# crmorton/Turbo-Whisper-Workspace

Hardware: AMD Instinct MI355X
Metric: real-time factor (audio-sec/wall-sec) Whisper-v3-turbo, 30s chunks, 1/2/4/8 GPU (higher is better)
Workload: dtype bf16; 1 GPU; whisper-large-v3-turbo bf16, batch=24 x 30s windows per GPU, greedy, 128 new tokens/window (EOS suppressed, one seek pass), timestamps on, language detected; collectives=none, global_batch=24, seq_len=3000, parallelism=chunk-dp1

## Files before the change

### turbo-whisper-workspace_amd/csrc/gemm.hip

```cpp
#include <algorithm>
#include <type_traits>

#include "tw_common.h"
#include "../../include/tw_whisper.h"

struct EpiArgs {
  void* out;
  int ldo;
  const float* bias;
  const float* aux;
  int aux_rows;
  int kv_S, kv_B, kv_D, kv_H;
  uint8_t* sout;
  int s_rows;
  int group_m;
};

__device__ inline void tw_tile_grouped(int wgid, int ntm, int ntn, int gm, int& tm, int& tn) {
  if (gm <= 1) {
    tm = wgid / ntn;
    tn = wgid - tm * ntn;
    return;
  }
  const int per = gm * ntn, g = wgid / per, first = g * gm;
// ... 222 lines not shown
        }
        continue;
      }
#pragma unroll
      for (int rr = 0; rr < 16; ++rr) {
        const int lr = rr * 4 + (lane >> 4);
        const int m = mrow0 + lr;
        float4 v = *(const float4*)(wimg + lr * GB_EPI_LD + rc);
        v.x += bias4.x; v.y += bias4.y; v.z += bias4.z; v.w += bias4.w;
        if (full) {
          if (m < M) epi_store4_pre<EPI>(ea, m, ncol0 + rc, v, ad[rr & 7]);
        } else if (m < M && ncol0 + rc < N) {
          epi_store4<EPI>(ea, m, ncol0 + rc, N, v);
        }
        if (rr < 8) ad[rr] = epi_addend<EPI>(ea, min(m + 32, M - 1), ncol0 + rc, full);
      }
    } else if constexpr (EPI == TW_EPI_BF16 || EPI == TW_EPI_GELU_BF16 || EPI == TW_EPI_CROSSKV) {
      const int rc8 = (lane & 7) * 8;
#pragma unroll 4
      for (int rr = 0; rr < 8; ++rr) {
        const int lr = rr * 8 + (lane >> 3);
        const int m = mrow0 + lr;
        float4 v0 = *(const float4*)(wimg + lr * GB_EPI_LD + rc8);
        float4 v1 = *(const float4*)(wimg + lr * GB_EPI_LD + rc8 + 4);
        v0.x += b8[0]; v0.y += b8[1]; v0.z += b8[2]; v0.w += b8[3];
        v1.x += b8[4]; v1.y += b8[5]; v1.z += b8[6]; v1.w += b8[7];
        if (m < M && ncol0 + rc8 < N) epi_store8<EPI>(ea, m, ncol0 + rc8, N, v0, v1);
      }
    } else {
#pragma unroll 4
      for (int rr = 0; rr < 16; ++rr) {
        const int lr = rr * 4 + (lane >> 4);
        const int m = mrow0 + lr;
        float4 v = *(const float4*)(wimg + lr * GB_EPI_LD + rc);
        v.x += bias4.x; v.y += bias4.y; v.z += bias4.z; v.w += bias4.w;
        if (m < M && ncol0 + rc < N) epi_store4<EPI>(ea, m, ncol0 + rc, N, v);
      }
    }
  }
}

template <int EPI>
__device__ inline void gemm_epi_128x64(const f32x4 (&acc)[8][4], float* wimg, int lane, int mw0, int ncol0, int M,
                                       int N, const EpiArgs& ea, bool interior = false) {
  const int fr = lane & 15, fq = lane >> 4;
  auto stage = [&](int half, float* w) {
    const int ib = 4 * half;
#pragma unroll
    for (int ii = 0; ii < 4; ++ii)
#pragma unroll
      for (int j = 0; j < 4; ++j)
#pragma unroll
        for (int r = 0; r < 4; ++r) w[(ii * 16 + fq * 4 + r) * GB_EPI_LD + j * 16 + fr] = acc[ib + ii][j][r];
  };
  gemm_epi_128x64_st<EPI>(stage, wimg, lane, mw0, ncol0, M, N, ea, interior);
}
template <int EPI, class Acc, class RowMap, class TCol>
__device__ inline void gemm_epi_tr(Acc acc, bf16_t* img, const float* bias_s, int lane, RowMap rowmap, TCol tcol, int n0,
                                   int M, int N, const EpiArgs& ea) {
  const int fr = lane & 15, fq = lane >> 4;
  float4 b4[4];
#pragma unroll
  for (int j = 0; j < 4; ++j)
    b4[j] = ea.bias ? *(const float4*)(bias_s + tcol(16 * j + 4 * fq)) : make_float4(0.f, 0.f, 0.f, 0.f);
  if constexpr (EPI == TW_EPI_BF16 || EPI == TW_EPI_GELU_BF16 || EPI == TW_EPI_CROSSKV) {
#pragma unroll
    for (int i = 0; i < 8; ++i) {
      const int row = 16 * i + fr;
#pragma unroll
      for (int j = 0; j < 4; ++j) {
        const f32x4 a = acc(i, j);
        float4 v = make_float4(a[0] + b4[j].x, a[1] + b4[j].y, a[2] + b4[j].z, a[3] + b4[j].w);
        if constexpr (EPI == TW_EPI_GELU_BF16) v = gelu_erf4(v);
        uint2 w;
        w.x = pack_bf16x2(v.x, v.y);
        w.y = pack_bf16x2(v.z, v.w);
        *(uint2*)(img + row * 64 + (((4 * j + fq) ^ (row & 15)) << 2)) = w;
      }
    }
    gb_epi_sync();
#pragma unroll 4
    for (int rr = 0; rr < 16; ++rr) {
      const int row = rr * 8 + (lane >> 3), p = lane & 7, g = row & 15;
      uint4 d = *(const uint4*)(img + row * 64 + ((p ^ (g >> 1)) << 3));
      if (g & 1) d = make_uint4(d.z, d.w, d.x, d.y);
      const int m = rowmap(row), n = n0 + tcol(8 * p);
      if (m >= M || n >= N) continue;
      if (n + 7 < N) {
        size_t idx;
        if constexpr (EPI == TW_EPI_CROSSKV) {
          const int D = ea.kv_D, S = ea.kv_S;
          const int l = n / (2 * D), rem = n - l * 2 * D;
          const int kv = rem / D, hd = rem - kv * D;
          const int b = m / S, s2 = m - b * S;
          idx = ((((size_t)(l * 2 + kv) * ea.kv_B + b) * ea.kv_H + (hd >> 6)) * S + s2) * 64 + (hd & 63);
        } else {
          idx = (size_t)m * ea.ldo + n;
        }
        tw_st_enc<gb_nt_bit(EPI)>((bf16_t*)ea.out + idx, d);
      } else {
        const uint32_t u[4] = {d.x, d.y, d.z, d.w};
        EpiArgs e2 = ea;
        e2.bias = nullptr;
        for (int e = 0; e < 8 && n + e < N; ++e) {
          const bf16_t h = (bf16_t)((u[e >> 1] >> (16 * (e & 1))) & 0xffffu);
          if constexpr (EPI == TW_EPI_CROSSKV) {
            epi_store<EPI>(e2, m, n + e, bf16_to_f32(h));
          } else {
            ((bf16_t*)ea.out)[(size_t)m * ea.ldo + n + e] = h;
          }
        }
      }
    }
  } else {
    constexpr bool PRE = EPI == TW_EPI_RESID_F32 || EPI == TW_EPI_GELU_POS_F32;
    float4 ad[2][4];
    auto load_ad = [&](int i, float4 (&dst)[4]) {
      const int m = min(rowmap(16 * i + fr), M - 1);
#pragma unroll
      for (int j = 0; j < 4; ++j) {
        const int n = n0 + tcol(16 * j + 4 * fq);
        dst[j] = epi_addend<EPI>(ea, m, n, n + 3 < N);
      }
    };
    if constexpr (PRE) load_ad(0, ad[0]);
#pragma unroll
    for (int i = 0; i < 8; ++i) {
      if constexpr (PRE) {
        if (i + 1 < 8) load_ad(i + 1, ad[(i + 1) & 1]);
      }
      const int m = rowmap(16 * i + fr);
#pragma unroll
      for (int j = 0; j < 4; ++j) {
        const f32x4 a = acc(i, j);
        const float4 v = make_float4(a[0] + b4[j].x, a[1] + b4[j].y, a[2] + b4[j].z, a[3] + b4[j].w);
        const int n = n0 + tcol(16 * j + 4 * fq);
        if (m >= M || n >= N) continue;
        if (n + 3 < N) {
          if constexpr (PRE) epi_store4_pre<EPI>(ea, m, n, v, ad[i & 1][j]);
          else epi_store4<EPI>(ea, m, n, N, v);
        } else {
          epi_store4<EPI>(ea, m, n, N, v);
        }
      }
    }
  }
}

__device__ inline void gemm_bias_load(const EpiArgs& ea, int n0, int N, float4& b) {
  const int c = n0 + 4 * (threadIdx.x & 63);
  if (ea.bias)
    b = make_float4(ea.bias[min(c, N - 1)], ea.bias[min(c + 1, N - 1)], ea.bias[min(c + 2, N - 1)],
                    ea.bias[min(c + 3, N - 1)]);
}

template <int EPI, bool TR>
__global__ __launch_bounds__(512, 1) void k_gemm_big(const bf16_t* __restrict__ A, const bf16_t* __restrict__ W,
                                                     int M, int N, int K, int lda, int ldw, EpiArgs ea) {
  __shared__ __attribute__((aligned(16))) bf16_t smem[8 * 64 * GB_EPI_LD * 2];
  const int tid = threadIdx.x, lane = tid & 63, wid = tid >> 6;
  const int ntm = (M + GB_BM - 1) / GB_BM, ntn = (N + GB_BN - 1) / GB_BN;
  const int nwg = ntm * ntn;
  const int orig = blockIdx.x;
  const int q8 = nwg / 8, r8 = nwg % 8, xcd = orig % 8;
  const int wgid = (xcd < r8 ? xcd * (q8 + 1) : r8 * (q8 + 1) + (xcd - r8) * q8) + orig / 8;
  int tm, tn;
  tw_tile_grouped(wgid, ntm, ntn, ea.group_m, tm, tn);
  const int m0 = tm * GB_BM, n0 = tn * GB_BN;

  const bf16_t* ga[4];
  const bf16_t* gw[4];
#pragma unroll
  for (int i = 0; i < 4; ++i) {
    const int row = 8 * (4 * wid + i) + (lane >> 3);
    const int ch = (lane & 7) ^ gb_swz(row);
    ga[i] = A + (size_t)min(m0 + row, M - 1) * lda + ch * 8;
    gw[i] = W + (size_t)min(n0 + row, N - 1) * ldw + ch * 8;
  }
  auto stage = [&](int buf, int k0) {
    bf16_t* As = smem + buf * 2 * GB_BM * GB_BK;
    bf16_t* Ws = As + GB_BM * GB_BK;
#pragma unroll
    for (int i = 0; i < 4; ++i) {
      const int rb = 8 * (4 * wid + i) * GB_BK;
      __builtin_amdgcn_global_load_lds((const void*)(ga[i] + k0), (lds_void_t*)(As + rb), 16, 0, 0);
      __builtin_amdgcn_global_load_lds((const void*)(gw[i] + k0), (lds_void_t*)(Ws + rb), 16, 0, 0);
    }
  };

  const int wr = wid >> 2, wc = wid & 3;
  const int fr = lane & 15, fq = lane >> 4;
  f32x4 acc[8][4];
#pragma unroll
  for (int i = 0; i < 8; ++i)
#pragma unroll
    for (int j = 0; j < 4; ++j) acc[i][j] = (f32x4){0.f, 0.f, 0.f, 0.f};

  const int nk = K / GB_BK;
  float* bias_s = (float*)(smem + 4 * GB_BM * GB_BK);
  float4 bl = make_float4(0.f, 0.f, 0.f, 0.f);
  stage(0, 0);
  if (TR && wid == 0) gemm_bias_load(ea, n0, N, bl);
  if (TR && wid == 0) {
    asm volatile("s_waitcnt vmcnt(0)" ::: "memory");
    *(float4*)(bias_s + 4 * lane) = bl;
  }
  __syncthreads();
  for (int kt = 0; kt < nk; ++kt) {
    const int cur = kt & 1;
    if (kt + 1 < nk) stage(cur ^ 1, (kt + 1) * GB_BK);
    const bf16_t* As = smem + cur * 2 * GB_BM * GB_BK;
    const bf16_t* Ws = As + GB_BM * GB_BK;
#pragma unroll
    for (int kk = 0; kk < 2; ++kk) {
      const int kc = 4 * kk + fq;
      bf16x8 bfr[4];
#pragma unroll
      for (int j = 0; j < 4; ++j) {
        const int col = wc * 64 + j * 16 + fr;
        bfr[j] = *(const bf16x8*)(Ws + col * GB_BK + ((kc ^ gb_swz(col)) << 3));
      }
#pragma unroll
      for (int i = 0; i < 8; ++i) {
        const int row = wr * 128 + i * 16 + fr;
        const bf16x8 af = *(const bf16x8*)(As + row * GB_BK + ((kc ^ gb_swz(row)) << 3));
#pragma unroll
        for (int j = 0; j < 4; ++j) {
          if constexpr (TR) acc[i][j] = __builtin_amdgcn_mfma_f32_16x16x32_bf16(bfr[j], af, acc[i][j], 0, 0, 0);
          else acc[i][j] = __builtin_amdgcn_mfma_f32_16x16x32_bf16(af, bfr[j], acc[i][j], 0, 0, 0);
        }
      }
    }
    __syncthreads();
  }

  if constexpr (TR) {
    gemm_epi_tr<EPI>([&](int i, int j) { return acc[i][j]; }, smem + wid * (128 * 64), bias_s, lane,
                     [&](int lr) { return m0 + wr * 128 + lr; }, [&](int lc) { return wc * 64 + lc; }, n0, M, N, ea);
  } else {
    gemm_epi_128x64<EPI>(acc, (float*)smem + wid * (64 * GB_EPI_LD), lane, m0 + wr * 128, n0 + wc * 64, M, N, ea,
                         m0 + GB_BM <= M && n0 + GB_BN <= N);
  }
}

__device__ inline __amdgpu_buffer_rsrc_t tw_uniform_rsrc(const void* p, int bytes) {
  const unsigned long long a = (unsigned long long)p;
  const unsigned lo = __builtin_amdgcn_readfirstlane((unsigned)a), hi = __builtin_amdgcn_readfirstlane((unsigned)(a >> 32));
  return __builtin_amdgcn_make_buffer_rsrc((void*)(((unsigned long long)hi << 32) | lo), 0,
                                           __builtin_amdgcn_readfirstlane(bytes), 0x00020000);
}

#ifdef TW_GEMM_PROBE
#define TW_PROBE_SLOTS 16
__device__ unsigned long long tw_probe_ts[32768 * TW_PROBE_SLOTS];
#define TW_PROBE(slot)                                                                                     \
  do {                                                                                                     \
    if (threadIdx.x == 0) tw_probe_ts[blockIdx.x * TW_PROBE_SLOTS + (slot)] = __builtin_amdgcn_s_memrealtime(); \
  } while (0)
#define TW_PROBE_CLK(slot)                                                                                 \
  do {                                                                                                     \
    if (threadIdx.x == 0) tw_probe_ts[blockIdx.x * TW_PROBE_SLOTS + (slot)] = __builtin_amdgcn_s_memtime();  \
  } while (0)
__device__ inline void tw_probe_ids() {
  if (threadIdx.x == 0) {
    unsigned hw, xcc;
    asm volatile("s_getreg_b32 %0, hwreg(HW_REG_HW_ID)" : "=s"(hw));
    asm volatile("s_getreg_b32 %0, hwreg(HW_REG_XCC_ID)" : "=s"(xcc));
    tw_probe_ts[blockIdx.x * TW_PROBE_SLOTS + 6] = hw;
    tw_probe_ts[blockIdx.x * TW_PROBE_SLOTS + 7] = xcc;
  }
}
extern "C" int tw_gemm_probe_read(unsigned long long* host, int nwg) {
  return (int)hipMemcpyFromSymbol(host, HIP_SYMBOL(tw_probe_ts), (size_t)nwg * TW_PROBE_SLOTS * 8, 0,
                                  hipMemcpyDeviceToHost);
}
#define TW_PROBE_W(slot)                              \
  do {                                                \
    asm volatile("s_waitcnt vmcnt(0) lgkmcnt(0)" ::: "memory"); \
    TW_PROBE(slot);                                   \
  } while (0)
#define TW_PROBE_END()                                \
  do {                                                \
    asm volatile("s_waitcnt vmcnt(0)" ::: "memory"); \
    __syncthreads();                                  \
    TW_PROBE(3);                                      \
  } while (0)
#else
#define TW_PROBE(slot) do {} while (0)
#define TW_PROBE_CLK(slot) do {} while (0)
#define TW_PROBE_END() do {} while (0)
#define TW_PROBE_W(slot) do {} while (0)
__device__ inline void tw_probe_ids() {}
#endif

template <int N>
__device__ inline void p8_vmcnt() {
  if constexpr (N == 0) asm volatile("s_waitcnt vmcnt(0)" ::: "memory");
  else if constexpr (N == 2) asm volatile("s_waitcnt vmcnt(2)" ::: "memory");
  else if constexpr (N == 4) asm volatile("s_waitcnt vmcnt(4)" ::: "memory");
  else if constexpr (N == 5) asm volatile("s_waitcnt vmcnt(5)" ::: "memory");
  else static_assert(N == 0, "unsupported vmcnt");
}

template <int EPI, bool TR>
__global__ __launch_bounds__(512, 1) void k_gemm_8p(const bf16_t* __restrict__ A, const bf16_t* __restrict__ W,
                                                    int M, int N, int K, int lda, int ldw, EpiArgs ea) {
  __shared__ __attribute__((aligned(16))) bf16_t smem[8 * 64 * GB_EPI_LD * 2];
  constexpr int HT = 128 * GB_BK;
  TW_PROBE(0);
  TW_PROBE_CLK(4);
  tw_probe_ids();
  const int tid = threadIdx.x, lane = tid & 63, wid = tid >> 6;
  const int ntm = (M + GB_BM - 1) / GB_BM, ntn = (N + GB_BN - 1) / GB_BN;
  const int nwg = ntm * ntn;
  const int orig = blockIdx.x;
  const int q8 = nwg / 8, r8 = nwg % 8, xcd = orig % 8;
  const int wgid = (xcd < r8 ? xcd * (q8 + 1) : r8 * (q8 + 1) + (xcd - r8) * q8) + orig / 8;
  int tm, tn;
  tw_tile_grouped(wgid, ntm, ntn, ea.group_m, tm, tn);
  const int m0 = tm * GB_BM, n0 = tn * GB_BN;
  const int wr = wid >> 2, wc = wid & 3;
  const int fr = lane & 15, fq = lane >> 4;

  __amdgpu_buffer_rsrc_t rs[4];
#pragma unroll
  for (int h = 0; h < 4; ++h) {
    const int r0 = (h < 2 ? m0 : n0) + 128 * (h & 1), lim = h < 2 ? M : N, ld = h < 2 ? lda : ldw;
    const int rows = max(0, min(128, lim - r0));
    rs[h] = tw_uniform_rsrc((h < 2 ? A : W) + (size_t)r0 * ld, rows ? ((rows - 1) * ld + K) * 2 : 0);
  }
  unsigned voff[2][2];
#pragma unroll
  for (int i = 0; i < 2; ++i) {
    const int row = 8 * (2 * wid + i) + (lane >> 3);
    const int ch = (lane & 7) ^ gb_swz(row);
    voff[0][i] = (unsigned)(row * lda + ch * 8) * 2u;
    voff[1][i] = (unsigned)(row * ldw + ch * 8) * 2u;
  }
  auto stage = [&](int buf, int h, int k0) {
    bf16_t* dst = smem + (buf * 4 + h) * HT;
#pragma unroll
    for (int i = 0; i < 2; ++i)
      __builtin_amdgcn_raw_ptr_buffer_load_lds(rs[h], (lds_void_t*)(dst + 8 * (2 * wid + i) * GB_BK), 16,
                                               voff[h >> 1][i], (unsigned)k0 * 2u, 0, 0);
  };

  bf16x8 af[4][2], bfr[2][2];
  auto readA = [&](int buf, int mh) {
    const bf16_t* As = smem + (buf * 4 + mh) * HT;
#pragma unroll
    for (int i = 0; i < 4; ++i)
#pragma unroll
      for (int kk = 0; kk < 2; ++kk) {
        const int row = 64 * wr + 16 * i + fr, kc = 4 * kk + fq;
        af[i][kk] = *(const bf16x8*)(As + row * GB_BK + ((kc ^ gb_swz(row)) << 3));
      }
  };
  auto readB = [&](int buf, int nh) {
    const bf16_t* Bs = smem + (buf * 4 + 2 + nh) * HT;
#pragma unroll
    for (int j = 0; j < 2; ++j)
#pragma unroll
      for (int kk = 0; kk < 2; ++kk) {
        const int row = 32 * wc + 16 * j + fr, kc = 4 * kk + fq;
        bfr[j][kk] = *(const bf16x8*)(Bs + row * GB_BK + ((kc ^ gb_swz(row)) << 3));
      }
  };
  f32x4 acc[2][2][4][2];
#pragma unroll
  for (int a = 0; a < 2; ++a)
#pragma unroll
    for (int b = 0; b < 2; ++b)
#pragma unroll
      for (int i = 0; i < 4; ++i)
#pragma unroll
        for (int j = 0; j < 2; ++j) acc[a][b][i][j] = (f32x4){0.f, 0.f, 0.f, 0.f};
  auto mfma_q = [&](auto MH, auto NH) {
    constexpr int mh = decltype(MH)::value, nh = decltype(NH)::value;
    __builtin_amdgcn_s_barrier();
    asm volatile("s_waitcnt lgkmcnt(0)" ::: "memory");
    __builtin_amdgcn_s_setprio(1);
#pragma unroll
    for (int kk = 0; kk < 2; ++kk)
#pragma unroll
      for (int i = 0; i < 4; ++i)
#pragma unroll
        for (int j = 0; j < 2; ++j)
          acc[mh][nh][i][j] = TR ? __builtin_amdgcn_mfma_f32_16x16x32_bf16(bfr[j][kk], af[i][kk], acc[mh][nh][i][j], 0, 0, 0)
                                 : __builtin_amdgcn_mfma_f32_16x16x32_bf16(af[i][kk], bfr[j][kk], acc[mh][nh][i][j], 0, 0, 0);
    __builtin_amdgcn_s_setprio(0);
    __builtin_amdgcn_s_barrier();
  };
  using I0 = std::integral_constant<int, 0>;
  using I1 = std::integral_constant<int, 1>;

  const int nk = K / GB_BK;
  float* bias_s = (float*)(smem + 8 * HT);
  float4 bl = make_float4(0.f, 0.f, 0.f, 0.f);
#pragma unroll
  for (int h = 0; h < 4; ++h) stage(0, h, 0);
  if (TR && wid == 0) gemm_bias_load(ea, n0, N, bl);
  asm volatile("s_waitcnt vmcnt(0)" ::: "memory");
  if (TR && wid == 0) *(float4*)(bias_s + 4 * lane) = bl;
  if (TR) asm volatile("s_waitcnt lgkmcnt(0)" ::: "memory");
  __builtin_amdgcn_s_barrier();
  TW_PROBE(1);
  if (wr == 1) __builtin_amdgcn_s_barrier();
  auto ktile = [&](int t, auto NXT) {
    constexpr bool nxt = decltype(NXT)::value;
    const int buf = t & 1, nb = buf ^ 1, kn = (t + 1) * GB_BK;
    readB(buf, 0);
    __builtin_amdgcn_sched_barrier(0);
    readA(buf, 0);
    if constexpr (nxt) {
      stage(nb, 0, kn);
      p8_vmcnt<4>();
    } else {
      p8_vmcnt<2>();
    }
    mfma_q(I0{}, I0{});
    readB(buf, 1);
    if constexpr (nxt) {
      stage(nb, 2, kn);
      p8_vmcnt<4>();
    } else {
      p8_vmcnt<0>();
    }
    mfma_q(I0{}, I1{});
    readA(buf, 1);
    if constexpr (nxt) stage(nb, 3, kn);
    mfma_q(I1{}, I1{});
    readB(buf, 0);
    if constexpr (nxt) {
      stage(nb, 1, kn);
      p8_vmcnt<4>();
    }
    mfma_q(I1{}, I0{});
  };
  using BT = std::integral_constant<bool, true>;
  using BF = std::integral_constant<bool, false>;
  for (int t = 0; t + 1 < nk; ++t) ktile(t, BT{});
  ktile(nk - 1, BF{});
  if (wr == 0) __builtin_amdgcn_s_barrier();
  __syncthreads();
  TW_PROBE(2);
  TW_PROBE_CLK(5);
  if constexpr (TR) {
    TW_PROBE_W(8);
    gemm_epi_tr<EPI>([&](int i, int j) { return acc[i >> 2][j >> 1][i & 3][j & 1]; }, smem + wid * (128 * 64), bias_s,
                     lane, [&](int lr) { return m0 + 128 * (lr >> 6) + 64 * wr + (lr & 63); },
                     [&](int lc) { return 128 * (lc >> 5) + 32 * wc + (lc & 31); }, n0, M, N, ea);
    TW_PROBE_END();
    return;
  }

  const int rc = (lane & 7) * 8;
  const int ncol = n0 + (rc < 32 ? 32 * wc + rc : 128 + 32 * wc + rc - 32);
  float4 b0 = make_float4(0.f, 0.f, 0.f, 0.f), b1 = b0;
  if (ea.bias) {
    b0.x = ea.bias[min(ncol, N - 1)];
    b0.y = ea.bias[min(ncol + 1, N - 1)];
    b0.z = ea.bias[min(ncol + 2, N - 1)];
    b0.w = ea.bias[min(ncol + 3, N - 1)];
    b1.x = ea.bias[min(ncol + 4, N - 1)];
    b1.y = ea.bias[min(ncol + 5, N - 1)];
    b1.z = ea.bias[min(ncol + 6, N - 1)];
    b1.w = ea.bias[min(ncol + 7, N - 1)];
  }
  float* wimg = (float*)smem + wid * (64 * GB_EPI_LD);
  TW_PROBE_W(8);
  constexpr bool PRE = EPI == TW_EPI_RESID_F32 || EPI == TW_EPI_GELU_POS_F32;
  const bool full = ncol + 7 < N;
#pragma unroll
  for (int mh = 0; mh < 2; ++mh) {
    const int mrow0 = m0 + 128 * mh + 64 * wr;
    float4 ad[4][2];
    if constexpr (PRE) {
#pragma unroll
      for (int q = 0; q < 4; ++q) {
        const int mq = min(mrow0 + q * 8 + (lane >> 3), M - 1);
        ad[q][0] = epi_addend<EPI>(ea, mq, ncol, full);
        ad[q][1] = epi_addend<EPI>(ea, mq, ncol + 4, full);
      }
    }
    if (mh) gb_epi_sync();
#pragma unroll
    for (int i = 0; i < 4; ++i)
#pragma unroll
      for (int nh = 0; nh < 2; ++nh)
#pragma unroll
        for (int j = 0; j < 2; ++j)
#pragma unroll
          for (int r = 0; r < 4; ++r)
            wimg[(i * 16 + fq * 4 + r) * GB_EPI_LD + nh * 32 + j * 16 + fr] = acc[mh][nh][i][j][r];
    gb_epi_sync();
    TW_PROBE_W(9 + 2 * mh);
#pragma unroll
    for (int rr = 0; rr < 8; ++rr) {
      const int lr = rr * 8 + (lane >> 3);
      const int m = mrow0 + lr;
      float4 v0 = *(const float4*)(wimg + lr * GB_EPI_LD + rc);
      float4 v1 = *(const float4*)(wimg + lr * GB_EPI_LD + rc + 4);
      v0.x += b0.x; v0.y += b0.y; v0.z += b0.z; v0.w += b0.w;
      v1.x += b1.x; v1.y += b1.y; v1.z += b1.z; v1.w += b1.w;
      if constexpr (PRE) {
        if (full) {
          if (m < M) {
            epi_store4_pre<EPI>(ea, m, ncol, v0, ad[rr & 3][0]);
            epi_store4_pre<EPI>(ea, m, ncol + 4, v1, ad[rr & 3][1]);
          }
        } else if (m < M && ncol < N) {
          epi_store8<EPI>(ea, m, ncol, N, v0, v1);
        }
        if (rr < 4) {
          const int mq = min(m + 32, M - 1);
          ad[rr][0] = epi_addend<EPI>(ea, mq, ncol, full);
          ad[rr][1] = epi_addend<EPI>(ea, mq, ncol + 4, full);
        }
      } else {
        if (m < M && ncol < N) epi_store8<EPI>(ea, m, ncol, N, v0, v1);
      }
    }
    TW_PROBE_W(10 + 2 * mh);
  }
  TW_PROBE_END();
}

__device__ inline void gb_read_rows4(const float* img, float4 (&v)[4][2]) {
  const unsigned a = (unsigned)(uintptr_t)(const __attribute__((address_space(3))) float*)img;
  asm volatile(
      "ds_read_b128 %0, %8\n\tds_read_b128 %1, %8 offset:16\n\t"
      "ds_read_b128 %2, %8 offset:%9\n\tds_read_b128 %3, %8 offset:%10\n\t"
      "ds_read_b128 %4, %8 offset:%11\n\tds_read_b128 %5, %8 offset:%12\n\t"
      "ds_read_b128 %6, %8 offset:%13\n\tds_read_b128 %7, %8 offset:%14\n\t"
      "s_waitcnt lgkmcnt(0)"
      : "=v"(v[0][0]), "=v"(v[0][1]), "=v"(v[1][0]), "=v"(v[1][1]), "=v"(v[2][0]), "=v"(v[2][1]), "=v"(v[3][0]),
        "=v"(v[3][1])
      : "v"(a), "i"(8 * GB_EPI_LD * 4), "i"(8 * GB_EPI_LD * 4 + 16), "i"(16 * GB_EPI_LD * 4),
        "i"(16 * GB_EPI_LD * 4 + 16), "i"(24 * GB_EPI_LD * 4), "i"(24 * GB_EPI_LD * 4 + 16)
      : "memory");
}

template <int EPI>
__global__ __launch_bounds__(512, 1) void k_gemm_8pp(const bf16_t* __restrict__ A, const bf16_t* __restrict__ W,
                                                     int M, int N, int K, int lda, int ldw, EpiArgs ea) {
  __shared__ __attribute__((aligned(16))) bf16_t smem[8 * 64 * GB_EPI_LD * 2];
  constexpr int HT = 128 * GB_BK;
  const int tid = threadIdx.x, lane = tid & 63, wid = tid >> 6;
  const int ntm = (M + GB_BM - 1) / GB_BM, ntn = (N + GB_BN - 1) / GB_BN;
  const int nwg = ntm * ntn;
  const int xcd = blockIdx.x % 8, slot = blockIdx.x / 8, S = gridDim.x / 8;
  const int q8 = nwg / 8, r8 = nwg % 8;
  const int cnt = q8 + (xcd < r8 ? 1 : 0);
  const int base = xcd < r8 ? xcd * (q8 + 1) : r8 * (q8 + 1) + (xcd - r8) * q8;
  if (slot >= cnt) return;
  const int wr = wid >> 2, wc = wid & 3;
  const int fr = lane & 15, fq = lane >> 4;
  float* const bias_sl = (float*)(smem + 4 * HT) + 8 * 32 * GB_EPI_LD;

  __amdgpu_buffer_rsrc_t rs[4];
  auto set_tile = [&](int tile, int& m0, int& n0) {
    int tm, tn;
    tw_tile_grouped(tile, ntm, ntn, ea.group_m, tm, tn);
    m0 = tm * GB_BM;
    n0 = tn * GB_BN;
#pragma unroll
    for (int h = 0; h < 4; ++h) {
      const int r0 = (h < 2 ? m0 : n0) + 128 * (h & 1), lim = h < 2 ? M : N, ld = h < 2 ? lda : ldw;
      const int rows = max(0, min(128, lim - r0));
      rs[h] = tw_uniform_rsrc((h < 2 ? A : W) + (size_t)r0 * ld, rows ? ((rows - 1) * ld + K) * 2 : 0);
    }
  };
  unsigned voff[2][2];
#pragma unroll
  for (int i = 0; i < 2; ++i) {
    const int row = 8 * (2 * wid + i) + (lane >> 3);
    const int ch = (lane & 7) ^ gb_swz(row);
    voff[0][i] = (unsigned)(row * lda + ch * 8) * 2u;
    voff[1][i] = (unsigned)(row * ldw + ch * 8) * 2u;
  }
  auto stage = [&](int buf, int h, int k0) {
    bf16_t* dst = smem + (buf * 4 + h) * HT;
#pragma unroll
    for (int i = 0; i < 2; ++i)
      __builtin_amdgcn_raw_ptr_buffer_load_lds(rs[h], (lds_void_t*)(dst + 8 * (2 * wid + i) * GB_BK), 16,
                                               voff[h >> 1][i], (unsigned)k0 * 2u, 0, 0);
  };
  auto stage_bias = [&](int sl, int n0) {
    if (ea.bias && wid == 0)
      __builtin_amdgcn_global_load_lds((const void*)(ea.bias + min(n0 + 4 * lane, N - 4)),
                                       (lds_void_t*)(bias_sl + 256 * sl), 16, 0, 0);
  };

  bf16x8 af[4][2], bfr[2][2];
  auto readA = [&](int buf, int mh) {
    const bf16_t* As = smem + (buf * 4 + mh) * HT;
#pragma unroll
    for (int i = 0; i < 4; ++i)
#pragma unroll
      for (int kk = 0; kk < 2; ++kk) {
        const int row = 64 * wr + 16 * i + fr, kc = 4 * kk + fq;
        af[i][kk] = *(const bf16x8*)(As + row * GB_BK + ((kc ^ gb_swz(row)) << 3));
      }
  };
  auto readB = [&](int buf, int nh) {
    const bf16_t* Bs = smem + (buf * 4 + 2 + nh) * HT;
#pragma unroll
    for (int j = 0; j < 2; ++j)
#pragma unroll
      for (int kk = 0; kk < 2; ++kk) {
        const int row = 32 * wc + 16 * j + fr, kc = 4 * kk + fq;
        bfr[j][kk] = *(const bf16x8*)(Bs + row * GB_BK + ((kc ^ gb_swz(row)) << 3));
      }
  };
  f32x4 acc[2][2][4][2];
  auto mfma_q = [&](auto MH, auto NH) {
    constexpr int mh = decltype(MH)::value, nh = decltype(NH)::value;
    __builtin_amdgcn_s_barrier();
    asm volatile("s_waitcnt lgkmcnt(0)" ::: "memory");
    __builtin_amdgcn_s_setprio(1);
#pragma unroll
    for (int kk = 0; kk < 2; ++kk)
#pragma unroll
      for (int i = 0; i < 4; ++i)
#pragma unroll
        for (int j = 0; j < 2; ++j)
          acc[mh][nh][i][j] = __builtin_amdgcn_mfma_f32_16x16x32_bf16(af[i][kk], bfr[j][kk], acc[mh][nh][i][j], 0, 0, 0);
    __builtin_amdgcn_s_setprio(0);
    __builtin_amdgcn_s_barrier();
  };
  using I0 = std::integral_constant<int, 0>;
  using I1 = std::integral_constant<int, 1>;
  auto ktile = [&](int t, auto NXT, auto FIRST) {
    constexpr bool nxt = decltype(NXT)::value, first = decltype(FIRST)::value;
    const int buf = t & 1, nb = buf ^ 1, kn = (t + 1) * GB_BK;
    readB(buf, 0);
    __builtin_amdgcn_sched_barrier(0);
    readA(buf, 0);
    if constexpr (nxt) {
      stage(nb, 0, kn);
      if constexpr (!first) p8_vmcnt<4>();
    } else if constexpr (!first) {
      p8_vmcnt<2>();
    }
    mfma_q(I0{}, I0{});
    readB(buf, 1);
    if constexpr (nxt) {
      stage(nb, 2, kn);
      if constexpr (!first) p8_vmcnt<4>();
    } else if constexpr (!first) {
      p8_vmcnt<0>();
    }
    mfma_q(I0{}, I1{});
    readA(buf, 1);
    if constexpr (nxt) stage(nb, 3, kn);
    mfma_q(I1{}, I1{});
    readB(buf, 0);
    if constexpr (nxt) {
      stage(nb, 1, kn);
      p8_vmcnt<4>();
    }
    mfma_q(I1{}, I0{});
  };
  using BT = std::integral_constant<bool, true>;
  using BF = std::integral_constant<bool, false>;

  constexpr bool PRE = EPI == TW_EPI_RESID_F32 || EPI == TW_EPI_GELU_POS_F32;
  constexpr bool BF16OUT = EPI == TW_EPI_BF16 || EPI == TW_EPI_GELU_BF16 || EPI == TW_EPI_CROSSKV;
  auto epilogue = [&](int m0, int n0, const float* bias_s) {
    const int rc = (lane & 7) * 8;
    const int lcol = rc < 32 ? 32 * wc + rc : 128 + 32 * wc + rc - 32;
    const int ncol = n0 + lcol;
    float4 b0 = make_float4(0.f, 0.f, 0.f, 0.f), b1 = b0;
    if (ea.bias) {
      b0 = *(const float4*)(bias_s + lcol);
      b1 = *(const float4*)(bias_s + lcol + 4);
    }
    float* wimg = (float*)(smem + 4 * HT) + wid * (32 * GB_EPI_LD);
    const bool full = ncol + 7 < N;
    auto stage_q = [&](int q, float4 (&vv)[4][2]) {
      const int mh = q >> 1, ih = q & 1;
      if (q) gb_epi_sync();
#pragma unroll
      for (int ii = 0; ii < 2; ++ii)
#pragma unroll
        for (int nh = 0; nh < 2; ++nh)
#pragma unroll
          for (int j = 0; j < 2; ++j)
#pragma unroll
            for (int r = 0; r < 4; ++r)
              wimg[(ii * 16 + fq * 4 + r) * GB_EPI_LD + nh * 32 + j * 16 + fr] = acc[mh][nh][2 * ih + ii][j][r];
      gb_epi_sync();
      gb_read_rows4(wimg + (lane >> 3) * GB_EPI_LD + rc, vv);
    };
    if constexpr (PRE) {
      if (m0 + GB_BM <= M && n0 + GB_BN <= N) {
#pragma unroll
        for (int q = 0; q < 4; ++q) {
          const int mr = m0 + 128 * (q >> 1) + 64 * wr + 32 * (q & 1) + (lane >> 3);
          float4 ad[4][2];
#pragma unroll
          for (int rr = 0; rr < 4; ++rr) {
            ad[rr][0] = epi_addend<EPI>(ea, mr + rr * 8, ncol, true);
            ad[rr][1] = epi_addend<EPI>(ea, mr + rr * 8, ncol + 4, true);
          }
          float4 vv[4][2];
          stage_q(q, vv);
#pragma unroll
          for (int rr = 0; rr < 4; ++rr) {
            float4 v0 = vv[rr][0], v1 = vv[rr][1];
            v0.x += b0.x; v0.y += b0.y; v0.z += b0.z; v0.w += b0.w;
            v1.x += b1.x; v1.y += b1.y; v1.z += b1.z; v1.w += b1.w;
            epi_store4_pre<EPI>(ea, mr + rr * 8, ncol, v0, ad[rr][0]);
            epi_store4_pre<EPI>(ea, mr + rr * 8, ncol + 4, v1, ad[rr][1]);
          }
        }
        return;
      }
    }
#pragma unroll
    for (int q = 0; q < 4; ++q) {
      const int mh = q >> 1, ih = q & 1;
      const int mrow0 = m0 + 128 * mh + 64 * wr + 32 * ih;
      float4 ad[4][2];
      if constexpr (PRE) {
#pragma unroll
        for (int rr = 0; rr < 4; ++rr) {
          const int mq = min(mrow0 + rr * 8 + (lane >> 3), M - 1);
          ad[rr][0] = epi_addend<EPI>(ea, mq, ncol, full);
          ad[rr][1] = epi_addend<EPI>(ea, mq, ncol + 4, full);
        }
      }
      float4 vv[4][2];
      stage_q(q, vv);
#pragma unroll
      for (int rr = 0; rr < 4; ++rr) {
        const int lr = rr * 8 + (lane >> 3);
        const int m = mrow0 + lr;
        float4 v0 = vv[rr][0], v1 = vv[rr][1];
        v0.x += b0.x; v0.y += b0.y; v0.z += b0.z; v0.w += b0.w;
        v1.x += b1.x; v1.y += b1.y; v1.z += b1.z; v1.w += b1.w;
        if constexpr (PRE) {
          if (full) {
            if (m < M) {
              epi_store4_pre<EPI>(ea, m, ncol, v0, ad[rr][0]);
              epi_store4_pre<EPI>(ea, m, ncol + 4, v1, ad[rr][1]);
            }
          } else if (m < M && ncol < N) {
            epi_store8<EPI>(ea, m, ncol, N, v0, v1);
          }
        } else {
          if (m < M && ncol < N) epi_store8<EPI>(ea, m, ncol, N, v0, v1);
        }
      }
    }
  };

  const int nk = K / GB_BK;
  int local = slot, m0, n0;
  set_tile(base + local, m0, n0);
#pragma unroll
  for (int h = 0; h < 4; ++h) stage(0, h, 0);
  stage_bias(0, n0);
  asm volatile("s_waitcnt vmcnt(0)" ::: "memory");
  __builtin_amdgcn_s_barrier();
  if (wr == 1) __builtin_amdgcn_s_barrier();
  for (int it = 0;; ++it) {
#pragma unroll
    for (int a = 0; a < 2; ++a)
#pragma unroll
      for (int b = 0; b < 2; ++b)
#pragma unroll
        for (int i = 0; i < 4; ++i)
#pragma unroll
          for (int j = 0; j < 2; ++j) acc[a][b][i][j] = (f32x4){0.f, 0.f, 0.f, 0.f};
    if (nk == 1) {
      ktile(0, BF{}, BT{});
    } else {
      ktile(0, BT{}, BT{});
      for (int t = 1; t + 1 < nk; ++t) ktile(t, BT{}, BF{});
      ktile(nk - 1, BF{}, BF{});
    }
    if (wr == 0) __builtin_amdgcn_s_barrier();
    __syncthreads();
    const int nlocal = local + S;
    const bool has_next = nlocal < cnt;
    const int cm0 = m0, cn0 = n0;
    if (has_next) {
      set_tile(base + nlocal, m0, n0);
#pragma unroll
      for (int h = 0; h < 4; ++h) stage(0, h, 0);
      stage_bias((it + 1) & 1, n0);
    }
    epilogue(cm0, cn0, bias_sl + 256 * (it & 1));
    if (!has_next) break;
    if (BF16OUT && cm0 + GB_BM <= M && cn0 + GB_BN <= N)
      asm volatile("s_waitcnt vmcnt(16)" ::: "memory");
    else if (PRE && cm0 + GB_BM <= M && cn0 + GB_BN <= N)
// ... 1054 lines not shown
```

Measured before the change: 8170 audio-s/wall-s.

## Cap GEMM VGPRs, regroup LDS buffers, and make k-loop buffer indices compile-time

The 8-phase bf16 GEMM kernel gets an arch-VGPR cap attribute and makes the wave id scalar via readfirstlane. The LDS double buffers are regrouped so A and B halves sit together, and swizzled LDS read offsets are precomputed per lane. The k-loop is unrolled by two so the buffer index is a compile-time constant, with the prologue buffer chosen by nk parity. The epilogue also takes a fast unclamped path for bias loads and defers the GELU addend load for the first half, all to cut address arithmetic and register pressure, at the risk of spills under the tight VGPR cap.

```diff
diff --git a/turbo-whisper-workspace_amd/csrc/gemm.hip b/turbo-whisper-workspace_amd/csrc/gemm.hip
--- a/turbo-whisper-workspace_amd/csrc/gemm.hip
+++ b/turbo-whisper-workspace_amd/csrc/gemm.hip
@@ -548,15 +548,17 @@
   else static_assert(N == 0, "unsupported vmcnt");
 }
 
+#define TW_VGPR_CAP_192 __attribute__((amdgpu_num_vgpr(96)))
 template <int EPI, bool TR>
-__global__ __launch_bounds__(512, 1) void k_gemm_8p(const bf16_t* __restrict__ A, const bf16_t* __restrict__ W,
-                                                    int M, int N, int K, int lda, int ldw, EpiArgs ea) {
+__global__ __launch_bounds__(512, 1) TW_VGPR_CAP_192 void k_gemm_8p(const bf16_t* __restrict__ A,
+                                                                    const bf16_t* __restrict__ W, int M, int N, int K,
+                                                                    int lda, int ldw, EpiArgs ea) {
   __shared__ __attribute__((aligned(16))) bf16_t smem[8 * 64 * GB_EPI_LD * 2];
   constexpr int HT = 128 * GB_BK;
   TW_PROBE(0);
   TW_PROBE_CLK(4);
   tw_probe_ids();
-  const int tid = threadIdx.x, lane = tid & 63, wid = tid >> 6;
+  const int tid = threadIdx.x, lane = tid & 63, wid = __builtin_amdgcn_readfirstlane(tid >> 6);
   const int ntm = (M + GB_BM - 1) / GB_BM, ntn = (N + GB_BN - 1) / GB_BN;
   const int nwg = ntm * ntn;
   const int orig = blockIdx.x;
@@ -584,33 +586,38 @@
     voff[1][i] = (unsigned)(row * ldw + ch * 8) * 2u;
   }
   auto stage = [&](int buf, int h, int k0) {
-    bf16_t* dst = smem + (buf * 4 + h) * HT;
+    bf16_t* dst = smem + ((h >> 1) * 4 + buf * 2 + (h & 1)) * HT;
 #pragma unroll
     for (int i = 0; i < 2; ++i)
       __builtin_amdgcn_raw_ptr_buffer_load_lds(rs[h], (lds_void_t*)(dst + 8 * (2 * wid + i) * GB_BK), 16,
                                                voff[h >> 1][i], (unsigned)k0 * 2u, 0, 0);
   };
 
+  const int sw = (fr >> 1) & 7;
+  unsigned pa[2], pb[2];
+#pragma unroll
+  for (int kk = 0; kk < 2; ++kk) {
+    const unsigned ch = (unsigned)(((4 * kk + fq) ^ sw) << 4);
+    pa[kk] = (unsigned)(64 * wr + fr) * (GB_BK * 2) + ch;
+    pb[kk] = (unsigned)(4 * HT * 2) + (unsigned)(32 * wc + fr) * (GB_BK * 2) + ch;
+  }
+  const char* smem_b = (const char*)smem;
   bf16x8 af[4][2], bfr[2][2];
-  auto readA = [&](int buf, int mh) {
-    const bf16_t* As = smem + (buf * 4 + mh) * HT;
+  auto readA = [&](auto BUF, int mh) {
+    constexpr int buf = decltype(BUF)::value;
 #pragma unroll
     for (int i = 0; i < 4; ++i)
 #pragma unroll
-      for (int kk = 0; kk < 2; ++kk) {
-        const int row = 64 * wr + 16 * i + fr, kc = 4 * kk + fq;
-        af[i][kk] = *(const bf16x8*)(As + row * GB_BK + ((kc ^ gb_swz(row)) << 3));
-      }
-  };
-  auto readB = [&](int buf, int nh) {
-    const bf16_t* Bs = smem + (buf * 4 + 2 + nh) * HT;
+      for (int kk = 0; kk < 2; ++kk)
+        af[i][kk] = *(const bf16x8*)(smem_b + pa[kk] + ((buf * 2 + mh) * HT + 16 * i * GB_BK) * 2);
+  };
+  auto readB = [&](auto BUF, int nh) {
+    constexpr int buf = decltype(BUF)::value;
 #pragma unroll
     for (int j = 0; j < 2; ++j)
 #pragma unroll
-      for (int kk = 0; kk < 2; ++kk) {
-        const int row = 32 * wc + 16 * j + fr, kc = 4 * kk + fq;
-        bfr[j][kk] = *(const bf16x8*)(Bs + row * GB_BK + ((kc ^ gb_swz(row)) << 3));
-      }
+      for (int kk = 0; kk < 2; ++kk)
+        bfr[j][kk] = *(const bf16x8*)(smem_b + pb[kk] + ((buf * 2 + nh) * HT + 16 * j * GB_BK) * 2);
   };
   f32x4 acc[2][2][4][2];
 #pragma unroll
@@ -644,7 +651,7 @@
   float* bias_s = (float*)(smem + 8 * HT);
   float4 bl = make_float4(0.f, 0.f, 0.f, 0.f);
 #pragma unroll
-  for (int h = 0; h < 4; ++h) stage(0, h, 0);
+  for (int h = 0; h < 4; ++h) stage(nk & 1, h, 0);
   if (TR && wid == 0) gemm_bias_load(ea, n0, N, bl);
   asm volatile("s_waitcnt vmcnt(0)" ::: "memory");
   if (TR && wid == 0) *(float4*)(bias_s + 4 * lane) = bl;
@@ -652,9 +659,11 @@
   __builtin_amdgcn_s_barrier();
   TW_PROBE(1);
   if (wr == 1) __builtin_amdgcn_s_barrier();
-  auto ktile = [&](int t, auto NXT) {
+  auto ktile = [&](int t, auto BUF, auto NXT) {
     constexpr bool nxt = decltype(NXT)::value;
-    const int buf = t & 1, nb = buf ^ 1, kn = (t + 1) * GB_BK;
+    constexpr int nb = decltype(BUF)::value ^ 1;
+    const auto buf = BUF;
+    const int kn = (t + 1) * GB_BK;
     readB(buf, 0);
     __builtin_amdgcn_sched_barrier(0);
     readA(buf, 0);
@@ -685,10 +694,20 @@
   };
   using BT = std::integral_constant<bool, true>;
   using BF = std::integral_constant<bool, false>;
-  for (int t = 0; t + 1 < nk; ++t) ktile(t, BT{});
-  ktile(nk - 1, BF{});
+  int t = 0;
+  if (!(nk & 1)) {
+    ktile(0, I0{}, BT{});
+    t = 1;
+  }
+  for (; t + 1 < nk; t += 2) {
+    ktile(t, I1{}, BT{});
+    ktile(t + 1, I0{}, BT{});
+  }
+  do ktile(t, I1{}, BF{});
+  while (K < 0);
   if (wr == 0) __builtin_amdgcn_s_barrier();
   __syncthreads();
+  __builtin_amdgcn_sched_barrier(0);
   TW_PROBE(2);
   TW_PROBE_CLK(5);
   if constexpr (TR) {
@@ -704,14 +723,21 @@
   const int ncol = n0 + (rc < 32 ? 32 * wc + rc : 128 + 32 * wc + rc - 32);
   float4 b0 = make_float4(0.f, 0.f, 0.f, 0.f), b1 = b0;
   if (ea.bias) {
-    b0.x = ea.bias[min(ncol, N - 1)];
-    b0.y = ea.bias[min(ncol + 1, N - 1)];
-    b0.z = ea.bias[min(ncol + 2, N - 1)];
-    b0.w = ea.bias[min(ncol + 3, N - 1)];
-    b1.x = ea.bias[min(ncol + 4, N - 1)];
-    b1.y = ea.bias[min(ncol + 5, N - 1)];
-    b1.z = ea.bias[min(ncol + 6, N - 1)];
-    b1.w = ea.bias[min(ncol + 7, N - 1)];
+    const int nlast = N - 1 - ncol;
+    const float* bp = ea.bias + min(ncol, N - 1);
+    if (nlast >= 7) {
+      b0.x = bp[0]; b0.y = bp[1]; b0.z = bp[2]; b0.w = bp[3];
+      b1.x = bp[4]; b1.y = bp[5]; b1.z = bp[6]; b1.w = bp[7];
+    } else if (nlast >= 0) {
+      b0.x = bp[0];
+      b0.y = bp[min(1, nlast)];
+      b0.z = bp[min(2, nlast)];
+      b0.w = bp[min(3, nlast)];
+      b1.x = bp[min(4, nlast)];
+      b1.y = bp[min(5, nlast)];
+      b1.z = bp[min(6, nlast)];
+      b1.w = bp[min(7, nlast)];
+    }
   }
   float* wimg = (float*)smem + wid * (64 * GB_EPI_LD);
   TW_PROBE_W(8);
@@ -721,14 +747,16 @@
   for (int mh = 0; mh < 2; ++mh) {
     const int mrow0 = m0 + 128 * mh + 64 * wr;
     float4 ad[4][2];
-    if constexpr (PRE) {
+    auto load_ad = [&]() {
 #pragma unroll
       for (int q = 0; q < 4; ++q) {
         const int mq = min(mrow0 + q * 8 + (lane >> 3), M - 1);
         ad[q][0] = epi_addend<EPI>(ea, mq, ncol, full);
         ad[q][1] = epi_addend<EPI>(ea, mq, ncol + 4, full);
       }
-    }
+    };
+    const bool late = EPI == TW_EPI_GELU_POS_F32 && mh == 0;
+    if (PRE && !late) load_ad();
     if (mh) gb_epi_sync();
 #pragma unroll
     for (int i = 0; i < 4; ++i)
@@ -740,6 +768,7 @@
           for (int r = 0; r < 4; ++r)
             wimg[(i * 16 + fq * 4 + r) * GB_EPI_LD + nh * 32 + j * 16 + fr] = acc[mh][nh][i][j][r];
     gb_epi_sync();
+    if (PRE && late) load_ad();
     TW_PROBE_W(9 + 2 * mh);
 #pragma unroll
     for (int rr = 0; rr < 8; ++rr) {
```

Result: no change. 8152 audio-s/wall-s (-0.2%).
